# Hiroshiba/realtime-yukarin

Hardware: AMD Instinct MI355X
Metric: acoustic frames/s (stage1+stage2 fwd) @16kHz/5ms (higher is better)
Workload: dtype f32; 1 GPU; BASELINE config #3: stage-1 + stage-2 SR forward, buffer_time 0.5 s + 2x0.5 s convert_extra_time @16 kHz / 5 ms -> 300 real frames (384 padded) per window, 1 window(s) per GPU per step, SYN-64 random-init weights; model=SYN-64, frames=300, padded_frames=384, windows_per_gpu=1, lanes_per_gpu=2

## Files before the change

realtime_yukarin_amd/csrc/ry_exec.cpp:

```cpp
#include "ry_kernels.h"
#include "ry_plan.h"

static void fill_geom(RyConvGeom& g, const Layer& l, const LayerPlan& lp, int B, const float* s1, int C1, const float* s2, int C2) {
    memset(&g, 0, sizeof g);
    const TapTable t = make_taps(l);
    g.src1 = s1; g.src2 = s2; g.C1 = C1; g.C2 = C2; g.S1 = C1; g.S2 = C2;
    if (lp.path == PATH_IGEMM_BF16 && lp.x3) { g.C1 = 3 * C1; g.C2 = 3 * C2; g.S1 = 2 * C1; g.S2 = 2 * C2; }
    g.B = B; g.Hi = lp.Hi; g.Wi = lp.Wi; g.Ho = lp.Ho; g.Wo = lp.Wo;
    g.Hs = lp.Hi; g.Hos = lp.Ho;
    if (lp.crop_hi > 0) { g.Hi = lp.crop_hi; g.Ho = l.deconv ? 2 * lp.crop_hi : lp.crop_hi; }
    if (l.deconv) { g.Mh = g.Hi; g.Mw = lp.Wi; g.stride = 1; g.pad = 0; g.ostride = 2; }
    else { g.Mh = g.Ho; g.Mw = lp.Wo; g.stride = l.stride; g.pad = l.pad; g.ostride = 1; }
    g.nphases = t.nphases; g.ntaps = t.ntaps; g.N = l.cout; g.kw = l.deconv ? 2 : l.k; g.dil = l.deconv ? 1 : l.dil;
    const size_t esize = lp.path == PATH_IGEMM_BF16 ? 2 : 4;
    g.zoff1 = (unsigned)((size_t)B * lp.Hi * lp.Wi * g.S1 * esize); g.zoff2 = (unsigned)((size_t)B * lp.Hi * lp.Wi * g.S2 * esize);
    if (lp.crop_hi > 0 && lp.crop_lo > 0) {
        const size_t o1 = (size_t)lp.crop_lo * lp.Wi * g.S1 * esize, o2 = (size_t)lp.crop_lo * lp.Wi * g.S2 * esize;
        g.src1 = reinterpret_cast<const float*>(reinterpret_cast<const char*>(s1) + o1); g.zoff1 -= (unsigned)o1;
        if (s2) { g.src2 = reinterpret_cast<const float*>(reinterpret_cast<const char*>(s2) + o2); g.zoff2 -= (unsigned)o2; }
    }
    for (int ph = 0; ph < 4; ++ph) {
        g.pdy[ph] = (signed char)t.pdy[ph]; g.pdx[ph] = (signed char)t.pdx[ph];
        for (int tt = 0; tt < 16; ++tt) { g.tdy[ph][tt] = (signed char)t.dy[ph][tt]; g.tdx[ph][tt] = (signed char)t.dx[ph][tt]; }
    }
// ... 27 lines not shown
    const bool xl = os2_xl_ok(lp.os2_mt4, lp.os2_waves, lp.os2_depth);
    snprintf(nm, sizeof nm, "ry_c2d_os<%d,%d,%d,%d,%s>", lp.os2_mt4, lp.os2_nt4, lp.os2_waves, lp.os2_depth, xl ? "true" : "false");
    RY_TRY(Lc.begin(nm, l.name, lp.flops, lp.bytes, grid));
    bool done = false;
#define X(A, B_, C, D)                                                                                          \
    if (!done && lp.os2_mt4 == A && lp.os2_nt4 == B_ && lp.os2_waves == C && lp.os2_depth == D) {               \
        RY_LAUNCH((ry_c2d_os<A, B_, C, D, os2_xl_ok(A, C, D)>), grid, 64 * C, Lc.stream, p);                    \
        done = true;                                                                                            \
    }
    RY_OS2_CONFIGS(X)
#undef X
    if (!done) return fail(RY_EINVAL, "%s: no ry_c2d_os instantiation <%d,%d,%d,%d>", l.name, lp.os2_mt4, lp.os2_nt4, lp.os2_waves, lp.os2_depth);
    return Lc.end();
}

static int launch_rep_rows(Launcher& Lc, const Layer& l, const LayerPlan& lp, int B) {
    for (int copy = 0; copy < 2; ++copy) {
        if (copy == 0 ? !lp.w32 : !lp.w16) continue;
        const int px_bytes = copy == 0 ? 4 * l.cout : (lp.o16x3 ? 4 : 2) * l.cout;
        RyRepRowsParams q;
        q.base = copy == 0 ? lp.out : reinterpret_cast<float*>(lp.out16);
        q.row_f4 = lp.Wo * px_bytes / 16; q.img_f4 = (long long)lp.Ho * q.row_f4;
        q.src = lp.hole_lo - 1; q.dst0 = lp.hole_lo; q.nrows = lp.hole_n;
        dim3 rg((unsigned)((q.row_f4 + 255) / 256), (unsigned)lp.hole_n, (unsigned)B);
        RY_TRY(Lc.begin("ry_rep_rows", l.name, 0, (double)B * lp.hole_n * lp.Wo * px_bytes, rg));
        RY_LAUNCH(ry_rep_rows, rg, 256, Lc.stream, q);
        RY_TRY(Lc.end());
    }
    return RY_OK;
}

static size_t out_offset(const Layer& l, const LayerPlan& lp) {
    return lp.crop_hi > 0 ? (size_t)(l.deconv ? 2 : 1) * lp.crop_lo * lp.Wo * l.cout : 0;
}

static int launch_reduce(Launcher& Lc, const Layer& l, const LayerPlan& lp, int B, int Ho_run, float slope) {
    RyReduceParams r;
    const long long slab_stride = (long long)B * lp.Ho * lp.Wo * l.cout;
    const size_t ro = B == 1 ? out_offset(l, lp) : 0;
    r.slabs = lp.slabs + ro; r.splits = lp.splits; r.slab_stride = slab_stride;
    r.scale = l.scale; r.shift = l.shift; r.out = lp.w32 ? lp.out + ro : nullptr; r.out16 = lp.w16 ? lp.out16 + ro * (lp.o16x3 ? 2 : 1) : nullptr;
    r.x3 = lp.o16x3 ? 1 : 0;
    r.total = B == 1 ? (long long)Ho_run * lp.Wo * l.cout : slab_stride; r.N = l.cout;
    r.act = l.act; r.slope = slope;
    if (lp.splits >= 16 && r.total <= (1 << 20)) {
        dim3 rg((unsigned)((r.total / 4 + 63) / 64));
        RY_TRY(Lc.begin("ry_splitk_reduce_wide", l.name, 0, (double)r.total * 4 * (lp.splits + 1), rg));
// ... 147 lines not shown
    if (lp.path == PATH_WINO) return launch_wino(Lc, l, lp, B, s1, C1, s2, C2, slope);
    if (lp.path == PATH_IGEMM || lp.path == PATH_IGEMM_BF16) return launch_igemm(Lc, l, lp, B, s1, C1, s2, C2, slope);
    if (lp.path == PATH_FIRST) {
        RySrFirstParams p;
        p.x = s1; p.w = l.wdir; p.scale = l.scale; p.shift = l.shift; p.out16 = lp.w16 ? lp.out16 : nullptr;
        p.out = (lp.w32 || !p.out16) ? lp.out : nullptr;
        p.x3 = lp.o16x3 ? 1 : 0;
        p.B = B; p.H = lp.Hi; p.W = lp.Wi; p.N = l.cout; p.act = l.act; p.slope = slope;
        const int quads = l.cout / 4;
        p.qshift = -1;
        for (int sh = 0; sh < 16; ++sh) if ((1 << sh) == quads) p.qshift = sh;
        const long long per_row = (long long)((lp.Wi + 3) / 4) * quads;
        dim3 grid((unsigned)((per_row + 255) / 256), (unsigned)lp.Hi, (unsigned)B);
        if (grid.y > 65535u || grid.z > 65535u) return fail(RY_EINVAL, "%s: %u rows x %u windows exceed the grid limit", l.name, grid.y, grid.z);
        RY_TRY(Lc.begin("ry_sr_first", l.name, lp.flops, lp.bytes, grid));
        RY_LAUNCH((ry_sr_first<4>), grid, 256, Lc.stream, p);
        RY_TRY(Lc.end());
    } else if (lp.path == PATH_LAST) {
        RySrLastParams p;
        p.src1 = s1; p.src2 = s2; p.C1 = C1; p.C2 = C2; p.w = l.wdir; p.scale = l.scale; p.shift = l.shift;
        p.out = lp.out; p.B = B; p.H = lp.Hi; p.W = lp.Wi;
        p.rows_valid = lp.last_rows; p.out_cols = lp.last_cols; p.do_exp = lp.last_exp;
        p.row0 = lp.last_row0; p.out_rows = lp.last_out_rows > 0 ? lp.last_out_rows : lp.last_rows;
        const long long total = (long long)B * p.rows_valid * lp.Wi;
        dim3 grid((unsigned)((total + 7) / 8));
        if (C1 + C2 == 128 && lp.Wi % 16 == 0) {
            const long long strips = (long long)B * p.rows_valid * (lp.Wi / 16);
            p.xcd_band = 1;
            const long long nb = (strips + 7) / 8;
            dim3 sg((unsigned)(((nb + 7) / 8) * 8));
            RY_TRY(Lc.begin("ry_sr_last<false>", l.name, lp.flops, lp.bytes, sg));
            RY_LAUNCH(ry_sr_last<false>, sg, 256, Lc.stream, p);
        } else {
            RY_TRY(Lc.begin("ry_sr_last_gather", l.name, lp.flops, lp.bytes, grid));
            RY_LAUNCH(ry_sr_last_gather, grid, 256, Lc.stream, p);
        }
        RY_TRY(Lc.end());
    } else {
        RyDirectParams p;
        fill_geom(p.g, l, lp, B, s1, C1, s2, C2);
        const RyConvGeom& g = p.g;
        const int M = B * g.Mh * g.Mw;
        p.wd = l.wdir; p.scale = l.scale; p.shift = l.shift; p.out = lp.out; p.act = l.act; p.slope = slope;
        const long long total = (long long)M * l.cout;
        dim3 grid((unsigned)((total + 255) / 256), (unsigned)g.nphases);
        RY_TRY(Lc.begin("ry_conv_direct", l.name, lp.flops, lp.bytes, grid));
        RY_LAUNCH(ry_conv_direct, grid, 256, Lc.stream, p);
        RY_TRY(Lc.end());
    }
    return RY_OK;
}

static int launch_conv1d(Launcher& Lc, const Layer& l, const LayerPlan& lp, int B, const RySrc1d& sa, const RySrc1d& sb, float slope) {
// ... 526 lines not shown
    LayerForce f;
    f.path = path ? path : (l.wig ? PATH_IGEMM : PATH_DIRECT);
    if (path == PATH_WINO) {
        if (!wino_eligible(l, 2)) return fail(RY_EINVAL, "the Winograd path is the k4 s2 p1 layer with Cin %% 16 == 0 and Cout %% 64 == 0");
        f.wino_set = true; f.wino[0] = tile & 15; f.wino[1] = (tile >> 4) & 15; f.wino[2] = splits;
    } else if (path == PATH_OS2D) {
        if (!l.w2os) return fail(RY_EINVAL, "output-stationary path needs Cin %% 256 == 0 and Cout %% 4 == 0");
        f.os2_set = true; f.os2[0] = tile & 15; f.os2[1] = (tile >> 4) & 15; f.os2[2] = (tile >> 8) & 31; f.os2[3] = (tile >> 13) & 15;
    } else if (f.path == PATH_IGEMM || f.path == PATH_IGEMM_BF16 || f.path == PATH_IGEMM_X3) {
        f.kg = (tile & 16) ? 2 : ((tile & 32) ? 1 : 0);
        f.tile = tile & 15; f.splits = splits;
        if (f.tile < 0 || f.tile > TILE_96x128 || f.tile == 2) return fail(RY_EINVAL, "unknown tile");
        if (f.tile == TILE_128x64 ? Cout % 64 : (f.tile != 0 && Cout % 128)) return fail(RY_EINVAL, "tile does not divide Cout");
    }
    const int dtype = path == PATH_IGEMM_X3 ? 2 : path == PATH_IGEMM_BF16 ? 1 : 0;
    if (dtype != 0) RY_TRY(prepare_bf16(ctx, arena, l, dtype));
    RY_TRY(plan_s2_layer(ctx, arena, l, lp, B, dtype, f, false, false, 0));
    if (lp.path == PATH_WINO) {
        float* w = nullptr;
        RY_TRY(upload_wwin(ctx, arena, l, &w));
        lp.wwin = w;
    }
    lp.any_m_patch = true;
    const size_t out_elems = (size_t)B * lp.Ho * lp.Wo * Cout;
    float* dx = nullptr;
    RY_TRY(alloc_ztail(ctx, arena, &dx, (size_t)B * H * Wd * Cin));
    RY_TRY(arena.alloc(&lp.out, out_elems));
    RY_TRY(poison_fill(ctx, lp.out, out_elems));
    Launcher Lc{nullptr, ctx, ctx->stream, nullptr, nullptr};
    if (lp.path == PATH_LAST || (lp.path == PATH_OS2D && Cin % 512 == 0) || (lp.path == PATH_WINO && Cin % 32 == 0)) {
        const int Ch = Cin / 2;
        const size_t npix = (size_t)B * H * Wd;
        std::vector<float> ha(npix * Ch), hb(npix * Ch);
        for (size_t q = 0; q < npix; ++q) {
            memcpy(&ha[q * Ch], x + q * Cin, Ch * sizeof(float));
            memcpy(&hb[q * Ch], x + q * Cin + Ch, Ch * sizeof(float));
        }
        float* dx2 = nullptr;
        RY_TRY(alloc_ztail(ctx, arena, &dx2, npix * Ch));
        RT_TRY(rt::dmemset(dx + npix * Ch, 0, ZTAIL * sizeof(float), ctx->stream));
        RT_TRY(rt::h2d(dx, ha.data(), npix * Ch * sizeof(float), ctx->stream));
        RT_TRY(rt::h2d(dx2, hb.data(), npix * Ch * sizeof(float), ctx->stream));
        RT_TRY(rt::stream_sync(ctx->stream));
        l.cin_a = Ch; l.cin_b = Ch;
        RY_TRY(launch_conv2d(Lc, l, lp, B, dx, Ch, dx2, Ch, 0.2f));
    } else if (lp.path == PATH_IGEMM_BF16) {
        const size_t nx = (size_t)B * H * Wd * Cin;
// ... 25 lines not shown
```

realtime_yukarin_amd/csrc/ry_host.h:

```cpp
#pragma once
#include "ry_dev.h"

#include "../../include/ry355.h"

#include <cmath>
#include <cstdarg>
#include <cstdio>
#include <cstdlib>
#include <chrono>
#include <cstring>
#include <map>
#include <memory>
#include <string>
#include <tuple>
#include <vector>

namespace rt {
#ifdef RY_HOST_EMU
typedef int err_t;
static const char* err_str(err_t) { return "emu"; }
static err_t set_device(int) { return 0; }
static err_t device_count(int* n) { *n = 1; return 0; }
static err_t stream_create(ry_stream_t* s) { *s = (ry_stream_t)malloc(1); return *s ? 0 : 1; }
static err_t stream_destroy(ry_stream_t s) { free((void*)s); return 0; }
// ... 167 lines not shown

struct LayerPlan {
    int Hi = 1, Wi = 1, Ho = 1, Wo = 1;
    int splits = 1;
    long long slab_stride = 0;
    float* raw = nullptr;
    int os_cb = 0, os_tp = 0, os_kt = 0;
    int path = 0, tile = 0;
    bool any_m_patch = false;
    int os2_mt4 = 0, os2_nt4 = 0, os2_waves = 0, os2_depth = 0;
    int wino_cfg = 0, wino_mbw = 0;
    const float* wwin = nullptr;
    int kg = 1;
    float* out = nullptr;
    unsigned short* out16 = nullptr;
    bool w32 = true, w16 = false;
    bool x3 = false;
    bool o16x3 = false;
    float* slabs = nullptr;
    int hole_lo = 0, hole_n = 0;
    int crop_hi = 0;
    int crop_lo = 0;
    int last_rows = 0, last_cols = 0, last_exp = 0;
    int last_row0 = 0, last_out_rows = 0;
    double flops = 0, bytes = 0;
    double flops_exec = 0;
};

inline void keep_rows(int n_frames, int disc_front, int disc_back, int* k0, int* k1) {
    *k0 = disc_front < n_frames ? disc_front : 0;
    *k1 = n_frames - disc_back > *k0 ? n_frames - disc_back : n_frames;
}

struct Plan {
    int B = 0, T = 0;
    int mode = 0;
    int n_frames = 0;
    int disc_front = 0, disc_back = 0;
    Arena arena;
    std::vector<LayerPlan> lp;
    float* user_in = nullptr;
    float* user_out = nullptr;
    float* x_in = nullptr;
    size_t user_in_floats = 0, user_out_floats = 0;
    bool s1_os = false;
    bool s1_padfuse = false;
// ... 92 lines not shown
```

realtime_yukarin_amd/csrc/ry_kernels.h:

```cpp
#pragma once
#include "ry_dev.h"


RY_DEV float ry_act(float v, int act, float slope) {
    if (act == RY_ACT_LRELU) return v >= 0.f ? v : v * slope;
    if (act == RY_ACT_RELU) return v > 0.f ? v : 0.f;
    return v;
}
RY_DEV float ry_sigmoid(float v) { return 1.f / (1.f + expf(-v)); }

RY_DEV int ry_fdiv(int x, int d, float inv_d) {
    int q = (int)((float)x * inv_d);
    const int r = x - q * d;
    q += (r >= d) ? 1 : 0;
    q -= (r < 0) ? 1 : 0;
    return q;
}

RY_DEV void ry_keep2(float& a, float& b) {
#ifndef RY_HOST_EMU
    asm volatile("" : "+v"(a), "+v"(b));
#endif
}
RY_DEV int ry_bitrev(int v, int bits) {
// ... 1138 lines not shown
        if (p.out) ry_st4(p.out + oi, o);
        if (p.out16) {
            if (p.x3) ry_st4_bf16_x3(p.out16, ((size_t)b * p.H + y) * p.W + x0 + j, p.N, cq * 4, o);
            else ry_st4_bf16(p.out16 + oi, o);
        }
    }
}

struct RySrLastParams {
    const float* src1;
    const float* src2;
    int C1, C2;
    const float* w;
    const float* scale;
    const float* shift;
    float* out;
    int B, H, W;
    int rows_valid;
    int row0;
    int out_rows;
    int out_cols;
    int do_exp;
    int xcd_band;
};

RY_KERNEL(256) void ry_sr_last_gather(RySrLastParams p) {
    const int l = (int)threadIdx.x & 31;
    const long long pix = (long long)blockIdx.x * 8 + (threadIdx.x >> 5);
    const long long total = (long long)p.B * p.rows_valid * p.W;
    const bool live = pix < total;
    const long long pp = live ? pix : 0;
    const int x = (int)(pp % p.W);
    const int y = (int)((pp / p.W) % p.rows_valid) + p.row0;
    const int b = (int)(pp / ((long long)p.W * p.rows_valid));
    const int Ctot = p.C1 + p.C2;
    float acc = 0.f;
    if (live) {
        for (int t = 0; t < 9; ++t) {
            const int iy = y + t / 3 - 1, ix = x + t % 3 - 1;
            if ((unsigned)iy >= (unsigned)p.H || (unsigned)ix >= (unsigned)p.W) continue;
            const size_t ipx = ((size_t)b * p.H + iy) * p.W + ix;
            for (int c = l * 4; c < Ctot; c += 128) {
                const f32x4 v = (c < p.C1) ? ry_ld4(p.src1 + ipx * p.C1 + c) : ry_ld4(p.src2 + ipx * p.C2 + (c - p.C1));
                const f32x4 wv = ry_ld4(p.w + (size_t)t * Ctot + c);
                acc = fmaf(v[3], wv[3], fmaf(v[2], wv[2], fmaf(v[1], wv[1], fmaf(v[0], wv[0], acc))));
            }
        }
    }
    acc += ry_shfl_xor(acc, 16);
    acc += ry_shfl_xor(acc, 8);
    acc += ry_shfl_xor(acc, 4);
    acc += ry_shfl_xor(acc, 2);
    acc += ry_shfl_xor(acc, 1);
    if (live && l == 0) {
        float v = fmaf(acc, p.scale[0], p.shift[0]);
        if (p.do_exp) v = expf(v);
        float* o = p.out + ((size_t)b * p.out_rows + y) * p.out_cols;
        o[x] = v;
        if (x == p.W - 1 && p.out_cols > p.W) o[p.W] = v;
    }
}

template <bool X3>
RY_KERNEL(256, 2) void ry_sr_last(RySrLastParams p) {
    static_assert(!X3, "ry_sr_last reads fp32 sources only");
    constexpr int SW = 16;
    const int l = (int)threadIdx.x & 31;
    const int strips = p.W / SW;
    const long long total = (long long)p.B * p.rows_valid * strips;
    long long lb = (long long)blockIdx.x;
    if (p.xcd_band) {
        const long long nb = (total + 7) >> 3, per = (nb + 7) >> 3;
        lb = (long long)(blockIdx.x & 7) * per + (blockIdx.x >> 3);
        if (lb >= nb) return;
    }
    const long long sid = lb * 8 + (threadIdx.x >> 5);
    const bool live = sid < total;
    const long long ss = live ? sid : 0;
    const int x0 = (int)(ss % strips) * SW;
    const int y = (int)((ss / strips) % p.rows_valid) + p.row0;
    const int b = (int)(ss / ((long long)strips * p.rows_valid));
    const int c = l * 4;
    const bool first = c < p.C1;
    const int Cs = first ? p.C1 : p.C2;
    const float* src = first ? p.src1 : p.src2;
    const int cl = first ? c : c - p.C1;
    auto ldpx = [&](const float* row, int px) -> f32x4 { return ry_ld4(row + (size_t)px * Cs + cl); };
    float acc[SW + 2];
#pragma unroll
    for (int j = 0; j < SW + 2; ++j) acc[j] = 0.f;
    if (live) {
#pragma unroll
        for (int ky = 0; ky < 3; ++ky) {
            const int iy = y + ky - 1;
            const bool rok = (unsigned)iy < (unsigned)p.H;
            const int iyc = rok ? iy : y;
            const float rz = rok ? 1.f : 0.f;
            f32x4 w0 = ry_ld4(p.w + (size_t)(ky * 3 + 0) * 128 + c);
            f32x4 w1 = ry_ld4(p.w + (size_t)(ky * 3 + 1) * 128 + c);
            f32x4 w2 = ry_ld4(p.w + (size_t)(ky * 3 + 2) * 128 + c);
            w0 *= rz; w1 *= rz; w2 *= rz;
            const float* row = src + ((size_t)b * p.H + iyc) * p.W * Cs;
#pragma unroll
            for (int j = 1; j <= SW; ++j) {
                const f32x4 v = ldpx(row, x0 - 1 + j);
                acc[j + 1] += fmaf(v[3], w0[3], fmaf(v[2], w0[2], fmaf(v[1], w0[1], v[0] * w0[0])));
                acc[j]     += fmaf(v[3], w1[3], fmaf(v[2], w1[2], fmaf(v[1], w1[1], v[0] * w1[0])));
                acc[j - 1] += fmaf(v[3], w2[3], fmaf(v[2], w2[2], fmaf(v[1], w2[1], v[0] * w2[0])));
            }
            {
                const bool lok = x0 > 0, rgt = x0 + SW < p.W;
                const f32x4 vl = ldpx(row, lok ? x0 - 1 : x0);
                const f32x4 vr = ldpx(row, rgt ? x0 + SW : x0);
                const float zl = lok ? 1.f : 0.f, zr = rgt ? 1.f : 0.f;
                acc[1]  += zl * fmaf(vl[3], w0[3], fmaf(vl[2], w0[2], fmaf(vl[1], w0[1], vl[0] * w0[0])));
                acc[SW] += zr * fmaf(vr[3], w2[3], fmaf(vr[2], w2[2], fmaf(vr[1], w2[1], vr[0] * w2[0])));
            }
        }
    }
    float r8[8], r4[4], r2[2], r1;
    const bool h16 = (l & 16) != 0, h8 = (l & 8) != 0, h4 = (l & 4) != 0, h2 = (l & 2) != 0;
#pragma unroll
    for (int i = 0; i < 8; ++i) {
        const float lo = acc[1 + i], hi = acc[1 + i + 8];
        const float recv = ry_shfl_xor(h16 ? lo : hi, 16);
        r8[i] = (h16 ? hi : lo) + recv;
    }
#pragma unroll
    for (int i = 0; i < 4; ++i) {
        const float recv = ry_shfl_xor(h8 ? r8[i] : r8[i + 4], 8);
        r4[i] = (h8 ? r8[i + 4] : r8[i]) + recv;
    }
#pragma unroll
    for (int i = 0; i < 2; ++i) {
        const float recv = ry_shfl_xor(h4 ? r4[i] : r4[i + 2], 4);
        r2[i] = (h4 ? r4[i + 2] : r4[i]) + recv;
    }
    {
        const float recv = ry_shfl_xor(h2 ? r2[0] : r2[1], 2);
        r1 = (h2 ? r2[1] : r2[0]) + recv;
    }
    r1 += ry_shfl_xor(r1, 1);
    if (live && (l & 1) == 0) {
        const int col = (h16 ? 8 : 0) + (h8 ? 4 : 0) + (h4 ? 2 : 0) + (h2 ? 1 : 0);
        const int x = x0 + col;
        float v = fmaf(r1, p.scale[0], p.shift[0]);
        if (p.do_exp) v = expf(v);
        float* o = p.out + ((size_t)b * p.out_rows + y) * p.out_cols;
        o[x] = v;
        if (x == p.W - 1 && p.out_cols > p.W) o[p.W] = v;
    }
}

struct RySrc1d {
    const float* raw;
    const float* scale;
    const float* shift;
    long long slab_stride;
    int C;
    int Craw;
    int splits;
    int act;
};

RY_DEV float ry_src1d_load(const RySrc1d& s, size_t pix, int c, float slope) {
    const float* q = s.raw + pix * s.Craw + c;
    float v = q[0];
    for (int k = 1; k < s.splits; ++k) v += q[(size_t)k * (size_t)s.slab_stride];
    if (s.scale) v = fmaf(v, s.scale[c], s.shift[c]);
    if (s.act == RY_ACT_GLU) {
        const float* qg = q + s.C;
        float gte = qg[0];
        for (int k = 1; k < s.splits; ++k) gte += qg[(size_t)k * (size_t)s.slab_stride];
// ... 420 lines not shown
    float* out;
    float slope;
};

RY_KERNEL(256) void ry_materialize(RyMaterializeParams p) {
    const long long idx = (long long)blockIdx.x * 256 + threadIdx.x;
    if (idx >= p.npix * p.s.C) return;
    const int c = (int)(idx % p.s.C);
    const long long row = idx / p.s.C;
    const size_t pix = (size_t)((row / p.keep) * p.L + row % p.keep);
    p.out[idx] = ry_src1d_load(p.s, pix, c, p.slope);
}

struct RyPadRowsParams {
    const float* in;
    const float* minv;
    float* out;
    int rows_in, cols_in, rows_out, cols_out;
    int take_log;
    long long in_bstride, out_bstride;
    int minv_bstride;
};

struct RyRepRowsParams { float* base; long long img_f4; int row_f4, src, dst0, nrows; };
RY_KERNEL(256) void ry_rep_rows(RyRepRowsParams p) {
    const int i = (int)blockIdx.x * 256 + (int)threadIdx.x;
    if (i >= p.row_f4) return;
    f32x4* img = reinterpret_cast<f32x4*>(p.base) + (size_t)blockIdx.z * (size_t)p.img_f4;
    img[(size_t)(p.dst0 + (int)blockIdx.y) * p.row_f4 + i] = img[(size_t)p.src * p.row_f4 + i];
}

template <int G>
RY_KERNEL(16 * G) void ry_pad_min_rows(RyPadRowsParams p) {
    __shared__ float red[16 * G];
    const int tid = (int)threadIdx.x, cl = tid & 15, grp = tid >> 4;
    const int c = (int)blockIdx.x * 16 + cl;
    const float* in = p.in + (size_t)blockIdx.y * (size_t)p.in_bstride;
    float* out = p.out + (size_t)blockIdx.y * (size_t)p.out_bstride;
    const bool cin_ok = c < p.cols_in, cout_ok = c < p.cols_out;
    float m = INFINITY;
    const bool need_min = p.rows_out > p.rows_in;
    for (int r0 = grp; r0 < p.rows_in; r0 += 8 * G) {
        float v[8];
#pragma unroll
        for (int u = 0; u < 8; ++u) { const int r = r0 + G * u; v[u] = (cin_ok && r < p.rows_in) ? in[(size_t)r * p.cols_in + c] : INFINITY; }
#pragma unroll
        for (int u = 0; u < 8; ++u) {
            const int r = r0 + G * u;
            m = fminf(m, v[u]);
            if (cout_ok && r < p.rows_in && r < p.rows_out) out[(size_t)r * p.cols_out + c] = p.take_log ? logf(v[u]) : v[u];
        }
    }
// ... 23 lines not shown
```

realtime_yukarin_amd/csrc/ry_plan.cpp:

```cpp
#include "ry_plan.h"

static const int ENC_CH[8] = {1, 2, 4, 8, 8, 8, 8, 8};
static const int DEC_IN[7] = {8, 16, 16, 16, 16, 8, 4};
static const int DEC_OUT[7] = {8, 8, 8, 8, 4, 2, 1};

std::vector<Layer> build_topology(const ry_net_desc& d) {
    std::vector<Layer> L(16);
    const int B = d.base, e = d.extensive_layers;
    const int end_k = e > 0 ? 3 : 1;
    const int g = (d.glu && d.ndim == 1) ? 2 : 1;
    const int blk_act_e = g == 2 ? RY_ACT_GLU : RY_ACT_LRELU, blk_act_d = g == 2 ? RY_ACT_GLU : RY_ACT_RELU;
    auto nm = [](Layer& l, const char* p, int i) { snprintf(l.name, sizeof l.name, "%s/c%d", p, i); };
    {
        Layer& l = L[0]; nm(l, "encoder", 0);
        l.k = end_k; l.stride = 1; l.pad = end_k / 2; l.cin_a = d.in_ch; l.cout = B; l.src_a = -1; l.act = RY_ACT_LRELU;
    }
    for (int i = 1; i < 8; ++i) {
        Layer& l = L[i]; nm(l, "encoder", i);
        const bool down = i < e;
        l.k = down ? 4 : 1; l.stride = down ? 2 : 1; l.pad = down ? 1 : 0;
        l.cin_a = ENC_CH[i - 1] * B; l.cout = ENC_CH[i] * B * g; l.src_a = i - 1; l.bn = true; l.act = blk_act_e;
    }
    for (int j = 0; j < 7; ++j) {
        Layer& l = L[8 + j]; nm(l, "decoder", j);
// ... 239 lines not shown
    return RY_OK;
}
int alloc_ztail(ry_ctx* ctx, Arena& arena, float** p, size_t nfloats) {
    RY_TRY(arena.alloc(p, nfloats + ZTAIL));
    if (g_poison) RT_TRY(rt::dmemset(*p, 0xFF, nfloats * sizeof(float), ctx->stream));
    RT_TRY(rt::dmemset(*p + nfloats, 0, ZTAIL * sizeof(float), ctx->stream));
    RT_TRY(rt::stream_sync(ctx->stream));
    return RY_OK;
}

void tile_dims(int tile, int* bm, int* bn) {
    switch (tile) {
        case TILE_128x128: *bm = 128; *bn = 128; break;
        case TILE_64x128: *bm = 64; *bn = 128; break;
        case TILE_128x64: *bm = 128; *bn = 64; break;
        case TILE_96x128: *bm = 96; *bn = 128; break;
        default: *bm = 32; *bn = 128; break;
    }
}


static int g_s2_hole = 1;
static int g_s2_crop = 2;
static LayerForce g_force[16];
bool layer_plan_fixed(int i) { return g_force[i].fixed(); }
int g_x3_min_m = 128;
int g_autotune = 0;
int g_autotune_reps = 3, g_autotune_max = 0;
int g_autotune_pick = -1;
const char* tile_name(int tile, int kg, bool bf16, int patch) {
    {
        static std::map<int, std::string> names;
        const int key = ((tile * 4 + kg) * 2 + (bf16 ? 1 : 0)) * 4 + patch;
        auto it = names.find(key);
        if (it == names.end()) {
            int bm, bn; tile_dims(tile, &bm, &bn);
            const int wmv = (tile == TILE_128x128) ? 2 : (tile == TILE_128x64 ? 4 : 1), wnv = 4 / wmv;
            char buf[96];
            snprintf(buf, sizeof buf, "ry_igemm_ldsdma<%d,%d,%d,%d,%d,%s,%d>", bm, bn, wmv, wnv, kg == 2 ? 2 : 1, bf16 ? "true" : "false", patch);
            it = names.emplace(key, buf).first;
        }
        return it->second.c_str();
    }
}

static thread_local double g_plan_peak = 157.3e6;
// ... 346 lines not shown
            return fail(RY_EINVAL, "RY_OS2: no output-stationary slice %d:%d:%d:%d for %s", c[0], c[1], c[2], c[3], l.name);
        }
    }
    if (f.path ? f.path == PATH_WINO
               : lp.path == PATH_IGEMM && dtype == 0 && g_wino && wino_eligible(l, 2) && !(f.wino_set && f.wino[0] == 0) && !f.fixed()) {
        const int Mh = l.deconv ? lp.Hi : lp.Ho, Mw = l.deconv ? lp.Wi : lp.Wo;
        int c[3] = {f.wino[0], f.wino[1], f.wino[2]};
        const int npatches = (l.deconv ? 1 : 4) * (l.cin() / 16);
        if ((f.wino_set || M >= g_wino_min_m) && choose_wino(Mh, Mw, l.cout, t.nphases, npatches, B, &c[0], &c[1], &c[2])) {
            lp.path = PATH_WINO; lp.wino_cfg = c[0]; lp.wino_mbw = c[1]; lp.splits = c[2]; lp.kg = 1; lp.tile = 0;
        } else if (f.wino_set) {
            if (f.path) return fail(RY_EINVAL, "no Winograd plan %d:%d:%d for a %d x %d grid", c[0], c[1], c[2], Mh, Mw);
            return fail(RY_EINVAL, "RY_WINO: no Winograd plan %d:%d:%d for %s", c[0], c[1], c[2], l.name);
        }
    }
    if (lp.path == 0) {
        lp.path = f.path ? f.path : PATH_DIRECT; lp.splits = 1;
        if (!f.path && !l.deconv && l.k == 3 && l.stride == 1 && l.pad == 1) {
            if (l.src_a < 0 && l.cin() == 1 && l.cout % 4 == 0) lp.path = PATH_FIRST;
            if (out_layer && l.cout == 1 && l.cin() % 128 == 0 && l.cin_a % 4 == 0) lp.path = PATH_LAST;
        }
        if (lp.path == PATH_LAST) {
            lp.last_rows = lp.Ho;
            lp.last_cols = mode == 1 ? lp.Wo + 1 : lp.Wo;
            lp.last_exp = mode == 1;
        }
    }
    if (lp.splits > 1) {
        const size_t out_elems = (size_t)B * lp.Ho * lp.Wo * l.cout;
        RY_TRY(arena.alloc(&lp.slabs, out_elems * lp.splits));
        RY_TRY(poison_fill(ctx, lp.slabs, out_elems * lp.splits));
    }
    return RY_OK;
}

int build_plan(ry_net* net, Plan& P) {
    const ry_net_desc& d = net->desc;
    const int nd = d.ndim, B = P.B;
    P.lp.assign(16, LayerPlan());
    int H = nd == 2 ? P.T : 1, W = nd == 2 ? d.width : P.T;
    for (int i = 0; i < 16; ++i) {
        const Layer& l = net->layers[i];
        LayerPlan& lp = P.lp[i];
        int hi, wi;
        if (l.src_a < 0) { hi = H; wi = W; } else { hi = P.lp[l.src_a].Ho; wi = P.lp[l.src_a].Wo; }
        lp.Hi = hi; lp.Wi = wi;
        if (l.deconv) { lp.Ho = nd == 2 ? hi * 2 : 1; lp.Wo = wi * 2; }
        else {
// ... 109 lines not shown
        if (v[0] < 0 || v[1] < 0 || v[2] < 0 || v[3] < 0) return false;
        f.os2_set = true; f.os2[0] = v[0]; f.os2[1] = v[1]; f.os2[2] = v[2]; f.os2[3] = v[3];
        return true;
    }));
    return parse_force("RY_PLAN", "layer:tile:splits:kgroups[,...]", [](LayerForce& f, const int* v) {
        if (v[0] < 0 || v[0] > TILE_96x128 || v[0] == 2 || v[1] < 0 || v[2] < 0 || v[2] > 2) return false;
        f.tile = v[0]; f.splits = v[1]; f.kg = v[2];
        return true;
    });
}

int read_env_switches() {
    g_autotune = 0; g_autotune_reps = 3; g_autotune_max = 0; g_autotune_pick = -1;
    if (const char* e = getenv("RY_AUTOTUNE")) {
        int on = 0, reps = 3, mx = 0, pick = -1;
        if (sscanf(e, "%d:%d:%d:%d", &on, &reps, &mx, &pick) < 1) return fail(RY_EINVAL, "RY_AUTOTUNE: expected 1[:reps[:max[:pick]]]");
        g_autotune = on; g_autotune_reps = reps > 0 ? reps : 1; g_autotune_max = mx; g_autotune_pick = pick;
    }
    g_x3_min_m = 128; g_s2_crop = 2;
    if (const char* e = getenv("RY_X3_MINM")) g_x3_min_m = atoi(e);
    if (const char* e = getenv("RY_S2_CROP")) g_s2_crop = atoi(e);
    g_s2_hole = 1;
    if (const char* e = getenv("RY_S2_HOLE")) g_s2_hole = atoi(e);
    return read_plan_env();
}

unsigned short host_f2bf(float f) {
    unsigned u; memcpy(&u, &f, 4);
    if ((u & 0x7fffffffu) > 0x7f800000u) return (unsigned short)((u >> 16) | 0x40);
    u += 0x7fffu + ((u >> 16) & 1u);
    return (unsigned short)(u >> 16);
}

float host_bf2f(unsigned short h) { const unsigned u = (unsigned)h << 16; float f; memcpy(&f, &u, 4); return f; }

static void build_wig16(const Layer& l, const std::vector<float>& w32, std::vector<unsigned short>& out) {
    const TapTable t = make_taps(l);
    const int C = l.cin(), N = l.cout;
    const size_t outer = (size_t)t.nphases * (N / 64) * t.ntaps;
    out.assign(outer * (size_t)C * 64, 0);
    for (size_t o = 0; o < outer; ++o)
        for (int c = 0; c < C; ++c)
            for (int nl = 0; nl < 64; ++nl)
                out[(o * (C / 64) + c / 64) * 4096 + wig16_inblock(nl, c % 64)] = host_f2bf(w32[(o * (C / 32) + c / 32) * 2048 + wig_inblock(nl, c % 32)]);
}

// ... 35 lines not shown
```

realtime_yukarin_amd/csrc/ry_plan.h:

```cpp
#pragma once
#include "ry_dev.h"
#include "ry_host.h"

struct TapTable {
    int nphases = 1, ntaps = 1;
    int dy[4][16], dx[4][16], ky[4][16], kx[4][16], pdy[4], pdx[4];
};

static const size_t ZTAIL = 2048;

#define RY_OS2_CONFIGS(X)                                                                                              \
    X(1, 1, 4, 4) X(1, 1, 8, 4) X(1, 1, 8, 2) X(1, 1, 16, 2) X(2, 1, 4, 4) X(2, 1, 8, 4) X(2, 1, 8, 2) X(2, 1, 16, 2)     \
    X(3, 1, 4, 4) X(3, 1, 8, 4) X(3, 1, 8, 2) X(3, 1, 16, 2) X(4, 1, 4, 4) X(4, 1, 8, 4) X(4, 1, 8, 2) X(4, 1, 16, 2)     \
    X(6, 1, 4, 4) X(6, 1, 8, 2)                                                             \
    X(1, 2, 4, 4) X(1, 2, 8, 4) X(1, 2, 8, 2) X(1, 2, 16, 2) X(2, 2, 4, 4) X(2, 2, 8, 4) X(2, 2, 8, 2) X(2, 2, 16, 2)     \
    X(3, 2, 4, 4) X(3, 2, 8, 4) X(3, 2, 8, 2) X(3, 2, 16, 2) X(4, 2, 4, 4) X(4, 2, 8, 4) X(4, 2, 8, 2) X(4, 2, 16, 2)     \
    X(6, 2, 4, 4) X(6, 2, 8, 2)                                                                             \
    X(1, 4, 4, 4) X(1, 4, 8, 4) X(1, 4, 8, 2) X(1, 4, 16, 2) X(2, 4, 4, 4) X(2, 4, 8, 4) X(2, 4, 8, 2) X(2, 4, 16, 2)     \
    X(3, 4, 4, 4) X(3, 4, 8, 4) X(3, 4, 8, 2) X(4, 4, 4, 4) X(4, 4, 8, 2) X(6, 4, 4, 2)

static constexpr bool os2_xl_ok(int mt4, int waves, int depth) { return depth == 2 && mt4 * waves <= 32; }

struct LayerForce {
    int tile = 0, splits = 0, kg = 0;
// ... 4 lines not shown
};

struct WindowRows {
    int k0 = 0, k1 = 0;
    int crop_lo[16] = {}, crop_hi[16] = {}, hole_lo[16] = {}, hole_n[16] = {};
};

std::vector<Layer> build_topology(const ry_net_desc& d);
size_t ipow(size_t b, int e);
size_t layer_param_count(const Layer& l, int ndim);
int check_desc(const ry_net_desc* d);
TapTable make_taps(const Layer& l);
bool wino_eligible(const Layer& l, int ndim);
int prepare_layer(ry_ctx* ctx, Arena& arena, Layer& l, int ndim, float eps, const float* W, const float* b, const float* bn, bool want_os2 = false);
int prepare_bf16(ry_ctx* ctx, Arena& arena, Layer& l, int dtype);
int upload_wwin(ry_ctx* ctx, Arena& arena, const Layer& l, float** out);
int alloc_ztail(ry_ctx* ctx, Arena& arena, float** p, size_t nfloats);
int poison_fill(ry_ctx* ctx, float* p, size_t nfloats);
void tile_dims(int tile, int* bm, int* bn);
extern int g_x3_min_m;
extern int g_autotune;
extern int g_autotune_reps, g_autotune_max;
extern int g_autotune_pick;
bool layer_plan_fixed(int i);
const char* tile_name(int tile, int kg, bool bf16, int patch);
int tile_occ(int tile, int kg);
double est_time(long blocks, int bm, int bn, int s, int occ, int kg, int M, int N, int nk);
void choose_igemm(const Layer& l, int M, int nphases, int nk, int* tile, int* splits, int* kg, int bf16 = 0 );
bool choose_os2(int M, int N, int nphases, int U, int* mt4, int* nt4, int* waves, int* depth, double* cost_out = nullptr);
bool wino_cfg_dims(int cfg, int* wm, int* wn, int* nsl);
void wino_tile_hw(int cfg, int mbw, int* th, int* tw);
const char* wino_name(int cfg, int mode);
bool choose_wino(int Mh, int Mw, int N, int nphases, int npatches, int B, int* cfg, int* mbw, int* splits);
int c1d_mode(const Layer& l);
int c1d_tile_len(int mode);
int choose_splits_1d(const Layer& l, int B, int rows, int mode);
bool c1d_os_capable(const Layer& l);
void plan_s1_os(const Layer& l, LayerPlan& lp, int B);
bool plan_tile_rows(const LayerPlan& lp, int Mh, int Mw, int* th, int* tw_out = nullptr);
bool plan_hole_ok(const Layer& l, const LayerPlan& lp, int lo, int n);
int plan_s2_layer(ry_ctx* ctx, Arena& arena, const Layer& l, LayerPlan& lp, int B, int dtype, const LayerForce& f, bool src16, bool out_layer, int mode);
WindowRows plan_window_rows(const ry_net* net, const Plan& P);
inline bool plan_padfuse_now(const ry_net* net, const Plan& P) { return net->desc.ndim == 1 && P.s1_padfuse && P.n_frames <= 2048; }
int build_plan(ry_net* net, Plan& P);
int autotune_plan(ry_net* net, Plan& P);
int get_plan(ry_net* net, int B, int T, int mode, int n_frames, Plan** out);
// ... 7 lines not shown
```

Baseline: 382,600 frames/s.

## Band rows in SR last-layer conv and batch hole-row replication

The final SR 3x3 conv kernel now processes a band of several output rows per wavefront (default 5). It streams input rows with a one-row prefetch and rotating accumulators, so each input row is loaded once per band instead of three times, and weights are staged in LDS. The rep_rows kernel now writes several destination rows per block from a single source load, which cuts the block count. Both add more registers and serial work per thread, and the output allocation for the last layer is resized to last_cols.

```diff
diff --git a/realtime_yukarin_amd/csrc/ry_exec.cpp b/realtime_yukarin_amd/csrc/ry_exec.cpp
--- a/realtime_yukarin_amd/csrc/ry_exec.cpp
+++ b/realtime_yukarin_amd/csrc/ry_exec.cpp
@@ -73,7 +73,11 @@
         q.base = copy == 0 ? lp.out : reinterpret_cast<float*>(lp.out16);
         q.row_f4 = lp.Wo * px_bytes / 16; q.img_f4 = (long long)lp.Ho * q.row_f4;
         q.src = lp.hole_lo - 1; q.dst0 = lp.hole_lo; q.nrows = lp.hole_n;
-        dim3 rg((unsigned)((q.row_f4 + 255) / 256), (unsigned)lp.hole_n, (unsigned)B);
+        const long long pieces = (q.row_f4 + 255) / 256;
+        const long long want = (pieces * lp.hole_n * B + 63) / 64;
+        q.per = g_rep_rows_per > 0 ? g_rep_rows_per : (int)(want < 1 ? 1 : want);
+        if (q.per > lp.hole_n) q.per = lp.hole_n;
+        dim3 rg((unsigned)pieces, (unsigned)((lp.hole_n + q.per - 1) / q.per), (unsigned)B);
         RY_TRY(Lc.begin("ry_rep_rows", l.name, 0, (double)B * lp.hole_n * lp.Wo * px_bytes, rg));
         RY_LAUNCH(ry_rep_rows, rg, 256, Lc.stream, q);
         RY_TRY(Lc.end());
@@ -267,13 +271,15 @@
         p.out = lp.out; p.B = B; p.H = lp.Hi; p.W = lp.Wi;
         p.rows_valid = lp.last_rows; p.out_cols = lp.last_cols; p.do_exp = lp.last_exp;
         p.row0 = lp.last_row0; p.out_rows = lp.last_out_rows > 0 ? lp.last_out_rows : lp.last_rows;
+        p.xcd_band = 0; p.band_rows = 1;
         const long long total = (long long)B * p.rows_valid * lp.Wi;
         dim3 grid((unsigned)((total + 7) / 8));
         if (C1 + C2 == 128 && lp.Wi % 16 == 0) {
-            const long long strips = (long long)B * p.rows_valid * (lp.Wi / 16);
-            p.xcd_band = 1;
+            p.band_rows = lp.last_band_rows > 0 ? lp.last_band_rows : 1;
+            const long long strips = (long long)B * ((p.rows_valid + p.band_rows - 1) / p.band_rows) * (lp.Wi / 16);
+            p.xcd_band = lp.last_xcd_band;
             const long long nb = (strips + 7) / 8;
-            dim3 sg((unsigned)(((nb + 7) / 8) * 8));
+            dim3 sg((unsigned)(p.xcd_band ? ((nb + 7) / 8) * 8 : nb));
             RY_TRY(Lc.begin("ry_sr_last<false>", l.name, lp.flops, lp.bytes, sg));
             RY_LAUNCH(ry_sr_last<false>, sg, 256, Lc.stream, p);
         } else {
@@ -846,7 +852,7 @@
         lp.wwin = w;
     }
     lp.any_m_patch = true;
-    const size_t out_elems = (size_t)B * lp.Ho * lp.Wo * Cout;
+    const size_t out_elems = (size_t)B * lp.Ho * (lp.path == PATH_LAST ? lp.last_cols : lp.Wo) * Cout;
     float* dx = nullptr;
     RY_TRY(alloc_ztail(ctx, arena, &dx, (size_t)B * H * Wd * Cin));
     RY_TRY(arena.alloc(&lp.out, out_elems));
diff --git a/realtime_yukarin_amd/csrc/ry_host.h b/realtime_yukarin_amd/csrc/ry_host.h
--- a/realtime_yukarin_amd/csrc/ry_host.h
+++ b/realtime_yukarin_amd/csrc/ry_host.h
@@ -213,6 +213,7 @@
     int crop_hi = 0;
     int crop_lo = 0;
     int last_rows = 0, last_cols = 0, last_exp = 0;
+    int last_band_rows = 1, last_xcd_band = 1;
     int last_row0 = 0, last_out_rows = 0;
     double flops = 0, bytes = 0;
     double flops_exec = 0;
diff --git a/realtime_yukarin_amd/csrc/ry_kernels.h b/realtime_yukarin_amd/csrc/ry_kernels.h
--- a/realtime_yukarin_amd/csrc/ry_kernels.h
+++ b/realtime_yukarin_amd/csrc/ry_kernels.h
@@ -1184,6 +1184,7 @@
     int out_cols;
     int do_exp;
     int xcd_band;
+    int band_rows;
 };
 
 RY_KERNEL(256) void ry_sr_last_gather(RySrLastParams p) {
@@ -1223,13 +1224,28 @@
     }
 }
 
+RY_DEV void ry_sr_last_row(float* acc, const f32x4* v, f32x4 w0, f32x4 w1, f32x4 w2, float zl, float zr) {
+    constexpr int SW = 16;
+#pragma unroll
+    for (int j = 1; j <= SW; ++j) {
+        acc[j + 1] += fmaf(v[j][3], w0[3], fmaf(v[j][2], w0[2], fmaf(v[j][1], w0[1], v[j][0] * w0[0])));
+        acc[j]     += fmaf(v[j][3], w1[3], fmaf(v[j][2], w1[2], fmaf(v[j][1], w1[1], v[j][0] * w1[0])));
+        acc[j - 1] += fmaf(v[j][3], w2[3], fmaf(v[j][2], w2[2], fmaf(v[j][1], w2[1], v[j][0] * w2[0])));
+    }
+    const f32x4 vl = v[0], vr = v[SW + 1];
+    acc[1]  += zl * fmaf(vl[3], w0[3], fmaf(vl[2], w0[2], fmaf(vl[1], w0[1], vl[0] * w0[0])));
+    acc[SW] += zr * fmaf(vr[3], w2[3], fmaf(vr[2], w2[2], fmaf(vr[1], w2[1], vr[0] * w2[0])));
+}
+
 template <bool X3>
 RY_KERNEL(256, 2) void ry_sr_last(RySrLastParams p) {
     static_assert(!X3, "ry_sr_last reads fp32 sources only");
     constexpr int SW = 16;
     const int l = (int)threadIdx.x & 31;
     const int strips = p.W / SW;
-    const long long total = (long long)p.B * p.rows_valid * strips;
+    const int R = p.band_rows;
+    const int chunks = (p.rows_valid + R - 1) / R;
+    const long long total = (long long)p.B * chunks * strips;
     long long lb = (long long)blockIdx.x;
     if (p.xcd_band) {
         const long long nb = (total + 7) >> 3, per = (nb + 7) >> 3;
@@ -1240,77 +1256,85 @@
     const bool live = sid < total;
     const long long ss = live ? sid : 0;
     const int x0 = (int)(ss % strips) * SW;
-    const int y = (int)((ss / strips) % p.rows_valid) + p.row0;
-    const int b = (int)(ss / ((long long)strips * p.rows_valid));
+    const int y0 = (int)((ss / strips) % chunks) * R + p.row0;
+    const int yend = p.row0 + p.rows_valid, y1 = y0 + R < yend ? y0 + R : yend;
+    const int b = (int)(ss / ((long long)strips * chunks));
     const int c = l * 4;
     const bool first = c < p.C1;
     const int Cs = first ? p.C1 : p.C2;
     const float* src = first ? p.src1 : p.src2;
     const int cl = first ? c : c - p.C1;
-    auto ldpx = [&](const float* row, int px) -> f32x4 { return ry_ld4(row + (size_t)px * Cs + cl); };
-    float acc[SW + 2];
-#pragma unroll
-    for (int j = 0; j < SW + 2; ++j) acc[j] = 0.f;
-    if (live) {
-#pragma unroll
-        for (int ky = 0; ky < 3; ++ky) {
-            const int iy = y + ky - 1;
-            const bool rok = (unsigned)iy < (unsigned)p.H;
-            const int iyc = rok ? iy : y;
-            const float rz = rok ? 1.f : 0.f;
-            f32x4 w0 = ry_ld4(p.w + (size_t)(ky * 3 + 0) * 128 + c);
-            f32x4 w1 = ry_ld4(p.w + (size_t)(ky * 3 + 1) * 128 + c);
-            f32x4 w2 = ry_ld4(p.w + (size_t)(ky * 3 + 2) * 128 + c);
-            w0 *= rz; w1 *= rz; w2 *= rz;
-            const float* row = src + ((size_t)b * p.H + iyc) * p.W * Cs;
-#pragma unroll
-            for (int j = 1; j <= SW; ++j) {
-                const f32x4 v = ldpx(row, x0 - 1 + j);
-                acc[j + 1] += fmaf(v[3], w0[3], fmaf(v[2], w0[2], fmaf(v[1], w0[1], v[0] * w0[0])));
-                acc[j]     += fmaf(v[3], w1[3], fmaf(v[2], w1[2], fmaf(v[1], w1[1], v[0] * w1[0])));
-                acc[j - 1] += fmaf(v[3], w2[3], fmaf(v[2], w2[2], fmaf(v[1], w2[1], v[0] * w2[0])));
+    const bool lok = x0 > 0, rgt = x0 + SW < p.W;
+    const float zl = lok ? 1.f : 0.f, zr = rgt ? 1.f : 0.f;
+    const float* col = src + ((size_t)b * p.H * p.W + (size_t)(lok ? x0 - 1 : x0)) * Cs + cl;
+    const int o1 = lok ? 1 : 0, or_ = (rgt ? x0 + SW : x0) - (lok ? x0 - 1 : x0);
+    auto ldrow = [&](f32x4* v, int s) {
+        int r = s < y1 ? s : y1;
+        r = r < 0 ? 0 : (r > p.H - 1 ? p.H - 1 : r);
+        const float* row = col + (size_t)r * p.W * Cs;
+        v[0] = ry_ld4(row);
+#pragma unroll
+        for (int j = 1; j <= SW; ++j) v[j] = ry_ld4(row + (size_t)(o1 + j - 1) * Cs);
+        v[SW + 1] = ry_ld4(row + (size_t)or_ * Cs);
+    };
+    __shared__ float wlds[9 * 128];
+    for (int i = (int)threadIdx.x; i < 9 * 32; i += 256) ry_st4(wlds + i * 4, ry_ld4(p.w + (size_t)i * 4));
+    __syncthreads();
+    const float sc = p.scale[0], sh = p.shift[0];
+    float a0[SW + 2], a1[SW + 2], a2[SW + 2];
+#pragma unroll
+    for (int j = 0; j < SW + 2; ++j) a0[j] = a1[j] = a2[j] = 0.f;
+    f32x4 v[SW + 2], vn[SW + 2];
+#pragma unroll
+    for (int j = 0; j < SW + 2; ++j) v[j] = vn[j] = f32x4{0.f, 0.f, 0.f, 0.f};
+    if (live) ldrow(v, y0 - 1);
+    const bool h16 = (l & 16) != 0, h8 = (l & 8) != 0, h4 = (l & 4) != 0, h2 = (l & 2) != 0;
+    for (int it = 0; it < R + 2; ++it) {
+        const int s = y0 - 1 + it;
+        if (live && it < R + 1) ldrow(vn, s + 1);
+        if (live) {
+            const float rz = (unsigned)s < (unsigned)p.H ? 1.f : 0.f;
+            auto wt = [&](int t) -> f32x4 { return ry_ld4(wlds + t * 128 + c) * rz; };
+            if (it >= 2) ry_sr_last_row(a0, v, wt(6), wt(7), wt(8), zl, zr);
+            if (it >= 1 && it <= R) ry_sr_last_row(a1, v, wt(3), wt(4), wt(5), zl, zr);
+            if (it < R) ry_sr_last_row(a2, v, wt(0), wt(1), wt(2), zl, zr);
+        }
+        if (it >= 2) {
+            float r8[8], r4[4], r2[2], r1;
+#pragma unroll
+            for (int i = 0; i < 8; ++i) {
+                const float lo = a0[1 + i], hi = a0[1 + i + 8];
+                const float recv = ry_shfl_xor(h16 ? lo : hi, 16);
+                r8[i] = (h16 ? hi : lo) + recv;
+            }
+#pragma unroll
+            for (int i = 0; i < 4; ++i) {
+                const float recv = ry_shfl_xor(h8 ? r8[i] : r8[i + 4], 8);
+                r4[i] = (h8 ? r8[i + 4] : r8[i]) + recv;
+            }
+#pragma unroll
+            for (int i = 0; i < 2; ++i) {
+                const float recv = ry_shfl_xor(h4 ? r4[i] : r4[i + 2], 4);
+                r2[i] = (h4 ? r4[i + 2] : r4[i]) + recv;
             }
             {
-                const bool lok = x0 > 0, rgt = x0 + SW < p.W;
-                const f32x4 vl = ldpx(row, lok ? x0 - 1 : x0);
-                const f32x4 vr = ldpx(row, rgt ? x0 + SW : x0);
-                const float zl = lok ? 1.f : 0.f, zr = rgt ? 1.f : 0.f;
-                acc[1]  += zl * fmaf(vl[3], w0[3], fmaf(vl[2], w0[2], fmaf(vl[1], w0[1], vl[0] * w0[0])));
-                acc[SW] += zr * fmaf(vr[3], w2[3], fmaf(vr[2], w2[2], fmaf(vr[1], w2[1], vr[0] * w2[0])));
-            }
-        }
-    }
-    float r8[8], r4[4], r2[2], r1;
-    const bool h16 = (l & 16) != 0, h8 = (l & 8) != 0, h4 = (l & 4) != 0, h2 = (l & 2) != 0;
-#pragma unroll
-    for (int i = 0; i < 8; ++i) {
-        const float lo = acc[1 + i], hi = acc[1 + i + 8];
-        const float recv = ry_shfl_xor(h16 ? lo : hi, 16);
-        r8[i] = (h16 ? hi : lo) + recv;
-    }
-#pragma unroll
-    for (int i = 0; i < 4; ++i) {
-        const float recv = ry_shfl_xor(h8 ? r8[i] : r8[i + 4], 8);
-        r4[i] = (h8 ? r8[i + 4] : r8[i]) + recv;
-    }
-#pragma unroll
-    for (int i = 0; i < 2; ++i) {
-        const float recv = ry_shfl_xor(h4 ? r4[i] : r4[i + 2], 4);
-        r2[i] = (h4 ? r4[i + 2] : r4[i]) + recv;
-    }
-    {
-        const float recv = ry_shfl_xor(h2 ? r2[0] : r2[1], 2);
-        r1 = (h2 ? r2[1] : r2[0]) + recv;
-    }
-    r1 += ry_shfl_xor(r1, 1);
-    if (live && (l & 1) == 0) {
-        const int col = (h16 ? 8 : 0) + (h8 ? 4 : 0) + (h4 ? 2 : 0) + (h2 ? 1 : 0);
-        const int x = x0 + col;
-        float v = fmaf(r1, p.scale[0], p.shift[0]);
-        if (p.do_exp) v = expf(v);
-        float* o = p.out + ((size_t)b * p.out_rows + y) * p.out_cols;
-        o[x] = v;
-        if (x == p.W - 1 && p.out_cols > p.W) o[p.W] = v;
+                const float recv = ry_shfl_xor(h2 ? r2[0] : r2[1], 2);
+                r1 = (h2 ? r2[1] : r2[0]) + recv;
+            }
+            r1 += ry_shfl_xor(r1, 1);
+            const int y = s - 1;
+            if (live && y < y1 && (l & 1) == 0) {
+                const int colx = (h16 ? 8 : 0) + (h8 ? 4 : 0) + (h4 ? 2 : 0) + (h2 ? 1 : 0);
+                const int x = x0 + colx;
+                float o_ = fmaf(r1, sc, sh);
+                if (p.do_exp) o_ = expf(o_);
+                float* o = p.out + ((size_t)b * p.out_rows + y) * p.out_cols;
+                o[x] = o_;
+                if (x == p.W - 1 && p.out_cols > p.W) o[p.W] = o_;
+            }
+        }
+#pragma unroll
+        for (int j = 0; j < SW + 2; ++j) { a0[j] = a1[j]; a1[j] = a2[j]; a2[j] = 0.f; v[j] = vn[j]; }
     }
 }
 
@@ -1777,12 +1801,14 @@
     int minv_bstride;
 };
 
-struct RyRepRowsParams { float* base; long long img_f4; int row_f4, src, dst0, nrows; };
+struct RyRepRowsParams { float* base; long long img_f4; int row_f4, src, dst0, nrows, per; };
 RY_KERNEL(256) void ry_rep_rows(RyRepRowsParams p) {
     const int i = (int)blockIdx.x * 256 + (int)threadIdx.x;
     if (i >= p.row_f4) return;
     f32x4* img = reinterpret_cast<f32x4*>(p.base) + (size_t)blockIdx.z * (size_t)p.img_f4;
-    img[(size_t)(p.dst0 + (int)blockIdx.y) * p.row_f4 + i] = img[(size_t)p.src * p.row_f4 + i];
+    const f32x4 v = img[(size_t)p.src * p.row_f4 + i];
+    const int r0 = (int)blockIdx.y * p.per, r1 = r0 + p.per < p.nrows ? r0 + p.per : p.nrows;
+    for (int r = r0; r < r1; ++r) img[(size_t)(p.dst0 + r) * p.row_f4 + i] = v;
 }
 
 template <int G>
diff --git a/realtime_yukarin_amd/csrc/ry_plan.cpp b/realtime_yukarin_amd/csrc/ry_plan.cpp
--- a/realtime_yukarin_amd/csrc/ry_plan.cpp
+++ b/realtime_yukarin_amd/csrc/ry_plan.cpp
@@ -285,6 +285,9 @@
 
 static int g_s2_hole = 1;
 static int g_s2_crop = 2;
+static const int SR_LAST_ROWS = 5;
+static int g_sr_last_rows = 0, g_sr_last_band = 1, g_sr_last_wrap = 0;
+int g_rep_rows_per = 0;
 static LayerForce g_force[16];
 bool layer_plan_fixed(int i) { return g_force[i].fixed(); }
 int g_x3_min_m = 128;
@@ -677,8 +680,11 @@
         }
         if (lp.path == PATH_LAST) {
             lp.last_rows = lp.Ho;
-            lp.last_cols = mode == 1 ? lp.Wo + 1 : lp.Wo;
-            lp.last_exp = mode == 1;
+            const bool wrap = mode == 1 || (f.path == PATH_LAST && g_sr_last_wrap);
+            lp.last_cols = wrap ? lp.Wo + 1 : lp.Wo;
+            lp.last_exp = wrap;
+            lp.last_band_rows = g_sr_last_rows > 0 ? g_sr_last_rows : SR_LAST_ROWS;
+            lp.last_xcd_band = g_sr_last_band;
         }
     }
     if (lp.splits > 1) {
@@ -834,6 +840,14 @@
     if (const char* e = getenv("RY_S2_CROP")) g_s2_crop = atoi(e);
     g_s2_hole = 1;
     if (const char* e = getenv("RY_S2_HOLE")) g_s2_hole = atoi(e);
+    g_rep_rows_per = 0;
+    if (const char* e = getenv("RY_REP_ROWS")) g_rep_rows_per = atoi(e) > 0 ? atoi(e) : 0;
+    g_sr_last_rows = 0; g_sr_last_band = 1; g_sr_last_wrap = 0;
+    if (const char* e = getenv("RY_SR_LAST")) {
+        int r = 0, band = 1, wrap = 0;
+        if (sscanf(e, "%d:%d:%d", &r, &band, &wrap) < 1 || r < 0 || r > 4096) return fail(RY_EINVAL, "RY_SR_LAST: expected rows[:band[:wrap]], 0 <= rows <= 4096");
+        g_sr_last_rows = r; g_sr_last_band = band != 0; g_sr_last_wrap = wrap != 0;
+    }
     return read_plan_env();
 }
 
diff --git a/realtime_yukarin_amd/csrc/ry_plan.h b/realtime_yukarin_amd/csrc/ry_plan.h
--- a/realtime_yukarin_amd/csrc/ry_plan.h
+++ b/realtime_yukarin_amd/csrc/ry_plan.h
@@ -50,6 +50,7 @@
 extern int g_autotune;
 extern int g_autotune_reps, g_autotune_max;
 extern int g_autotune_pick;
+extern int g_rep_rows_per;
 bool layer_plan_fixed(int i);
 const char* tile_name(int tile, int kg, bool bf16, int patch);
 int tile_occ(int tile, int kg);
```

After: 379,500 frames/s. Within noise of the previous version (-0.8%).
